# etemesi254/zune-jpeg

Hardware: AMD Instinct MI355X
Metric: megapixels/sec decoded (IDCT->RGB), 4K 4:2:0 baseline (higher is better)
Workload: dtype i32

## Files before the change

zune-jpeg_amd/csrc/zj_device.h:

```cpp
#pragma once

#include <stdint.h>

#if defined(ZJ_EMU)
#define ZJ_DEV inline
#define ZJ_HD inline
#else
#include <hip/hip_runtime.h>
#define ZJ_DEV __device__ __forceinline__
#define ZJ_HD __host__ __device__ __forceinline__
#endif

namespace zj {

typedef uint16_t u16x2 __attribute__((vector_size(4)));
typedef int16_t s16x2 __attribute__((vector_size(4)));

#if defined(ZJ_EMU)
#define ZJ_GLOBAL_PTR(T, v) (reinterpret_cast<T*>(v))
#else
#define ZJ_GLOBAL_PTR(T, v) ((T*)(__attribute__((address_space(1))) T*)(v))
#endif

struct alignas(16) U4 { uint32_t x, y, z, w; };
// ... 1 lines not shown
typedef uint32_t V4 __attribute__((vector_size(16)));
#if defined(ZJ_ABLATION)
#define ZJ_ABL(debug, bit) ((debug) & (bit))
#define ZJ_PDBG(p) ((p).debug)
#else
#define ZJ_ABL(debug, bit) 0
#define ZJ_PDBG(p) 0
#endif
#ifndef ZJ_NT
#define ZJ_NT 4
#endif
#ifndef ZJ_SEAM_WB
#define ZJ_SEAM_WB 0
#endif
#ifndef ZJ_ROUND_ROT
#define ZJ_ROUND_ROT 1
#endif

#ifndef ZJ_CBYTE
#define ZJ_CBYTE 1
#endif
#ifndef ZJ_INTERIOR
#define ZJ_INTERIOR 1
#endif

ZJ_DEV uint32_t as_u32(u16x2 v) { uint32_t r; __builtin_memcpy(&r, &v, 4); return r; }
ZJ_DEV uint32_t as_u32(s16x2 v) { uint32_t r; __builtin_memcpy(&r, &v, 4); return r; }
ZJ_DEV u16x2 as_u16x2(uint32_t v) { u16x2 r; __builtin_memcpy(&r, &v, 4); return r; }
ZJ_DEV s16x2 as_s16x2(uint32_t v) { s16x2 r; __builtin_memcpy(&r, &v, 4); return r; }

#if !defined(ZJ_EMU)
extern "C" __device__ __attribute__((const)) int zj_llvm_mul_i24(int, int) __asm("llvm.amdgcn.mul.i24");
#endif
ZJ_DEV int32_t mul24(int32_t a, int32_t b)
{
#if defined(ZJ_EMU)
    int32_t a24 = (int32_t)((uint32_t)a << 8) >> 8, b24 = (int32_t)((uint32_t)b << 8) >> 8;
    return (int32_t)((uint32_t)a24 * (uint32_t)b24);
#else
    return zj_llvm_mul_i24(a, b);
#endif
}
ZJ_DEV int32_t wadd(int32_t a, int32_t b) { return (int32_t)((uint32_t)a + (uint32_t)b); }
ZJ_DEV int32_t wsub(int32_t a, int32_t b) { return (int32_t)((uint32_t)a - (uint32_t)b); }
ZJ_DEV int32_t mad24(int32_t a, int32_t b, int32_t c) { return wadd(mul24(a, b), c); }
ZJ_DEV int32_t wshl(int32_t a, int s) { return (int32_t)((uint32_t)a << s); }
// ... 283 lines not shown
ZJ_DEV PackedHalf idct_1d_dot(const uint32_t p04, const uint32_t p26, const uint32_t p13, const uint32_t p57, const int32_t bias)
{
    PackedHalf h;
    const int32_t t0 = dot2(p04, pk16(4096, 4096), bias);
    const int32_t t1 = dot2(p04, pk16(4096, -4096), bias);
    h.x0 = dot2(p26, pk16(5352, 2217), t0);
    h.x3 = dot2(p26, pk16(-5352, -2217), t0);
    h.x1 = dot2(p26, pk16(2217, -5350), t1);
    h.x2 = dot2(p26, pk16(-2217, 5350), t1);
    h.u3 = dot2(p57, pk16(3219, 1131), dot2z(p13, pk16(5683, 4816)));
    h.u2 = dot2(p57, pk16(-5681, -3218), dot2z(p13, pk16(4816, -1129)));
    h.u1 = dot2(p57, pk16(1132, 4816), dot2z(p13, pk16(3219, -5681)));
    h.u0 = dot2(p57, pk16(4816, -5680), dot2z(p13, pk16(1131, -3218)));
    return h;
}
ZJ_DEV void idct_1d_dot_add(const PackedHalf& h, int32_t o[8])
{
    o[0] = wadd(h.x0, h.u3); o[7] = wsub(h.x0, h.u3);
    o[1] = wadd(h.x1, h.u2); o[6] = wsub(h.x1, h.u2);
    o[2] = wadd(h.x2, h.u1); o[5] = wsub(h.x2, h.u1);
    o[3] = wadd(h.x3, h.u0); o[4] = wsub(h.x3, h.u0);
}

ZJ_DEV int classify_block(const uint32_t* w, const uint32_t* g)
{
    uint32_t any = w[0] & 0xffff0000u;
#pragma unroll
    for (int i = 1; i < 32; i++) any |= w[i];
    if (any == 0) return 0;
    int32_t bad = 0;
#pragma unroll
    for (int jj = 0; jj < 4; jj++) {
        uint32_t st = 0, sb = 0;
#pragma unroll
        for (int k = 0; k < 4; k++) st = sad_u16(w[4 * k + jj], 0x80008000u, st);
#pragma unroll
        for (int k = 4; k < 8; k++) sb = sad_u16(w[4 * k + jj], 0x80008000u, sb);
        const int32_t d = mad24((int32_t)g[4 + jj], (int32_t)sb, mad24((int32_t)g[jj], (int32_t)st, -(int32_t)g[8 + jj]));
        bad |= d;
    }
    return bad < 0 ? 2 : 1;
}

ZJ_DEV void idct_block_packed(const U4 raw[8], const uint32_t* qp, uint32_t out[16])
{
    const uint32_t* w = reinterpret_cast<const uint32_t*>(raw);
    uint32_t D[32];
#pragma unroll
// ... 132 lines not shown
    static constexpr int NT_BLK = (NBLK + 63) / 64 * 64;
    static constexpr int NT_MIN = (HS == 1 && VS == 1) ? (CHROMA ? ZJ_NT_MIN_444 : ZJ_NT_MIN_GRAY) : ((HS == 2 && VS == 1 && CHROMA) ? ZJ_NT_MIN_H : ((HS == 2 && VS == 2 && CHROMA) ? ZJ_NT_MIN_HV : ((HS == 1 && VS == 2 && CHROMA) ? ZJ_NT_MIN_V : 0)));
    static constexpr int NT = NT_BLK > NT_MIN ? NT_BLK : NT_MIN;
    static constexpr int NW = NT / 64;
    static constexpr int ROUND_ROT = (ZJ_ROUND_ROT && NITEMS % NT != 0 && NITEMS % NT <= 64 && NW > 1) ? 1 : 0;

    static constexpr int LUT_N = SH + 2;
    static constexpr int LUT_BYTES = ((2 * LUT_N * 2 + 15) / 16) * 16;
    static constexpr int HRAW = (CHROMA && HALO) ? 2 * 2 * CROWS : 0;
    static constexpr int HFIL = (CHROMA && HALO) ? 2 * 2 * SH : 0;
    static constexpr bool TSCAP = OUT == OUT_RGB || OUT == OUT_YCBCR || OUT == OUT_RGBA;
    static constexpr int PPI = OUT == OUT_RGBA ? 4 : 3;
    static constexpr int INPL = 64 / PPI * PPI;
    static constexpr int XSTAGE = ((64 * PPI - INPL) * 16 + 31) / 32 * 32;
    static constexpr bool HALO_PURE = CHROMA && HALO && (NYB + 2 * CBR * TWC) % 64 == 0 && 2 * CBR * 2 * 8 == 64;
    static constexpr int HALO_T0 = NYB + 2 * CBR * TWC;
#if defined(ZJ_EMU) && !defined(ZJ_EMU_REDO_ANY)
    static constexpr bool CBYTE_OUT = OUT == OUT_RGB || OUT == OUT_RGBA || OUT == OUT_RGB_CHW;
#else
    static constexpr bool CBYTE_OUT = true;
#endif
    static constexpr bool CBYTE = ZJ_CBYTE != 0 && CHROMA && HS == 2 && HALO_PURE && NGRP == 16 && NYB % 64 == 0 && CBYTE_OUT;
    static constexpr bool INTERIOR = ZJ_INTERIOR != 0 && CBYTE && TSCAP && NITEMS % NT == 0 && ROUND_ROT == 0;
    template <int GEN> struct L {
        static constexpr int YPX = GEN == GEN_PACKED ? 1 : 2;
        static constexpr bool CB = GEN == GEN_PACKED && CBYTE;
        static constexpr int CPX = CB ? 1 : 2;
        static constexpr int CPB = CPITCH * CPX;
        static constexpr int CPLANE = CROWS * CPB;
        static constexpr int CBYTES = CHROMA ? 2 * CPLANE + (HRAW + HFIL) * 2 : 0;
        static_assert(CBYTES % 16 == 0, "tables stay 16-byte aligned");
        static constexpr int C_OFF = GEN == GEN_PACKED ? (NITEMS + 63) / 64 * 64 * 16 : YSZ * 2;
        static constexpr int HRAW_OFF = C_OFF + 2 * CPLANE;
        static constexpr int HFIL_OFF = HRAW_OFF + HRAW * 2;
        static constexpr int TAB_OFF = C_OFF + CBYTES;
        static constexpr int LUT_OFF = TAB_OFF + TAB_BYTES;
        static constexpr int FLAG_OFF = LUT_OFF + LUT_BYTES;
        static constexpr int X_OFF = FLAG_OFF + 16;
        static constexpr int X_STAGE = TSCAP ? NW * XSTAGE : 0;
        static constexpr int X_HALO = HALO_PURE ? 8 * 80 * 4 : 0;
        static constexpr int BYTES = GEN == GEN_PACKED ? X_OFF + (X_STAGE > X_HALO ? X_STAGE : X_HALO) : FLAG_OFF;
        static_assert(C_OFF % 16 == 0 && TAB_OFF % 16 == 0, "16-byte alignment of the planes");
    };
    static constexpr int LDS_WIDE = L<GEN_WIDE>::BYTES;
    static constexpr int LDS_PACKED = L<GEN_PACKED>::BYTES > LDS_WIDE ? L<GEN_PACKED>::BYTES : LDS_WIDE;
    static constexpr int PIECES_PER_ROW = PPI * NGRP;
// ... 259 lines not shown
    }
    if (GEN == GEN_PACKED && tid == 0) *lds_flag<C>(lds) = 0;
}

ZJ_DEV void rows_to_bytes(const U4 px[8], uint32_t b[16])
{
#pragma unroll
    for (int r = 0; r < 8; r++) {
        b[2 * r] = perm(px[r].y, px[r].x, 0x06040200u);
        b[2 * r + 1] = perm(px[r].w, px[r].z, 0x06040200u);
    }
}
ZJ_DEV void bytes_to_rows(const uint32_t b[16], U4 px[8])
{
#pragma unroll
    for (int r = 0; r < 8; r++) {
        px[r].x = perm(0, b[2 * r], 0x0c010c00u); px[r].y = perm(0, b[2 * r], 0x0c030c02u);
        px[r].z = perm(0, b[2 * r + 1], 0x0c010c00u); px[r].w = perm(0, b[2 * r + 1], 0x0c030c02u);
    }
}

struct HaloLane { const int16_t* src; char* dst; int pitch; int comp; int hb; int j; bool last_col; };

template <class C>
ZJ_DEV HaloLane halo_locate(const Params& p, const TileId t, const int hl , char* lds)
{
    HaloLane H;
    H.hb = hl >> 3; H.j = hl & 7;
    H.comp = 1 + H.hb / (2 * C::CBR);
    const int brow = (H.hb / 2) % C::CBR, side = H.hb & 1;
    const int cbw = p.mcu_x, cb0 = t.tile * C::TWC;
    const int nvalid = (cbw - cb0) < C::TWC ? (cbw - cb0) : C::TWC;
    const int gcol = side == 0 ? (cb0 > 0 ? cb0 - 1 : cbw - 1) : (cb0 + nvalid < cbw ? cb0 + nvalid : 0);
    const long long blk = (long long)(t.strip * C::CBR + brow) * cbw + gcol;
    const int16_t* plane = H.comp == 1 ? t.cb : t.cr;
    H.src = plane + blk * 64 + H.j;
    H.dst = reinterpret_cast<char*>(lds_halo_raw<C, GEN_PACKED>(lds, H.comp, side, brow * 8));
    H.pitch = 2;
    H.last_col = side == 0;
    return H;
}
ZJ_DEV void halo_load(const HaloLane& H, int32_t s[8])
{
#pragma unroll
    for (int k = 0; k < 8; k++) s[k] = H.src[8 * k];
}
template <class C> ZJ_DEV int32_t* lds_halo_scratch(char* lds, const int hb) { return reinterpret_cast<int32_t*>(lds + C::template L<GEN_PACKED>::X_OFF) + 80 * hb; }

template <class C>
ZJ_DEV void halo_pass1(const HaloLane& H, const int32_t s[8], char* lds)
{
    const uint16_t* q = reinterpret_cast<const uint16_t*>(lds_tab<C, GEN_PACKED>(lds) + TAB_DW * H.comp);
    int32_t* sc = lds_halo_scratch<C>(lds, H.hb);
    int32_t any = H.j == 0 ? 0 : s[0];
    int32_t d[8], o[8];
#pragma unroll
// ... 30 lines not shown
        int32_t u3 = mul24(t1, 6149 + 4816 - 3685 - 1597);
        u3 = mad24(t7, 4816 - 3685, u3);
        u3 = mad24(t5, 4816 - 1597, u3);
        u3 = mad24(t3, 4816, u3);
        v = (H.last_col ? wsub(x0, u3) : wadd(x0, u3)) >> 17;
        v = v < 0 ? 0 : (v > 255 ? 255 : v);
    }
    *reinterpret_cast<int16_t*>(H.dst + i * H.pitch) = (int16_t)v;
}

template <class C, int HS, int VS, int GEN>
ZJ_DEV int halo_value(char* lds, const int comp, const int side, const int m, const bool wrap)
{
    const int16_t* raw = lds_halo_raw<C, GEN>(lds, comp, side, 0);
    if (VS == 2) {
        const int16_t* lut = lds_lut<C, GEN>(lds);
        const int i = m + 1 + (wrap ? (side == 0 ? -1 : 1) : 0);
        const int ra = lut[i] / C::template L<GEN>::CPB, rb = lut[C::LUT_N + i] / C::template L<GEN>::CPB;
        return tri1(raw[ra], raw[rb]);
    }
    const int r = side == 0 ? (wrap && m > 0 ? m - 1 : m) : (wrap && m < C::SH - 1 ? m + 1 : m);
    return raw[r];
}
template <class C, int HS, int VS>
ZJ_DEV void halo_filter(const Params& p, const TileId t, const int hl, char* lds)
{
    const int cbw = p.mcu_x, cb0 = t.tile * C::TWC;
    const bool left_wrap = cb0 == 0, right_wrap = cb0 + C::TWC >= cbw;
    for (int q = hl; q < C::HFIL; q += 64) {
        const int comp = 1 + q / (2 * C::SH), side = (q / C::SH) & 1, m = q % C::SH;
        *lds_halo_fil<C, GEN_PACKED>(lds, comp, side, m) = (int16_t)halo_value<C, HS, VS, GEN_PACKED>(lds, comp, side, m, side == 0 ? left_wrap : right_wrap);
    }
}

template <class C, int GEN, bool NEED_Y16>
ZJ_DEV void finish_block(const BlockLoc& L, const U4 raw[8], char* lds, const int debug = 0, const int clamp_dc = 0)
{
    if (!L.valid) return;
    const uint32_t* w = reinterpret_cast<const uint32_t*>(raw);
    const uint32_t* tab = lds_tab<C, GEN>(lds) + TAB_DW * L.comp;
    if (GEN == GEN_WIDE) {
        uint32_t any = w[0] & 0xffff0000u;
#pragma unroll
        for (int i = 1; i < 32; i++) any |= w[i];
        if (any != 0 && !ZJ_ABL(debug, 1)) {
            U4 px[8];
            idct_block(raw, reinterpret_cast<const uint16_t*>(tab), px);
            store_block(L, px);
        } else {
            store_splat(L, dc_only_value(w[0], (int32_t)(tab[0] & 0xffffu), clamp_dc));
        }
        return;
    }
    using LLp = typename C::template L<GEN_PACKED>;
    constexpr bool CB = LLp::CB;
    constexpr bool CONST_PITCH = C::HALO_PURE && (CB || C::TWY * LLp::YPX == LLp::CPB);
    BlockLoc Lc = L;
    if (CONST_PITCH) { Lc.pitch = LLp::CPB; Lc.halo = 0; }
    const int ypitch = CONST_PITCH ? C::TWY * LLp::YPX : L.pitch;
    int cls = classify_block(w, tab + 32);
    if (ZJ_ABL(debug, 1)) cls = 0;
    if (cls == 0) {
        const uint32_t v = dc_only_value(w[0], (int32_t)(tab[0] & 0xffffu), clamp_dc);
        if (L.comp != 0 && !CB) { store_splat(Lc, v); return; }
        if ((L.comp != 0 || NEED_Y16) && (v & 0xffffu) > 255u) *lds_flag<C>(lds) = 1;
        const uint32_t b = (v & 0xffu) * 0x01010101u;
        const U2 row = {b, b};
        if (L.comp != 0) {
#pragma unroll
            for (int r = 0; r < 8; r++) *reinterpret_cast<U2*>(Lc.dst + r * Lc.pitch) = row;
            return;
        }
#pragma unroll
        for (int r = 0; r < 8; r++) *reinterpret_cast<U2*>(Lc.dst + r * ypitch) = row;
        return;
    }
    auto emit = [&](const uint32_t* b) {
        if (L.comp == 0) {
#pragma unroll
            for (int r = 0; r < 8; r++) { const U2 row = {b[2 * r], b[2 * r + 1]}; *reinterpret_cast<U2*>(Lc.dst + r * ypitch) = row; }
        } else if (CB) {
#pragma unroll
            for (int r = 0; r < 8; r++) { const U2 row = {b[2 * r], b[2 * r + 1]}; *reinterpret_cast<U2*>(Lc.dst + r * Lc.pitch) = row; }
// ... 174 lines not shown
        prev = (uint32_t)__builtin_amdgcn_update_dpp((int)pl, (int)a1, 0x111, 0xf, 0xf, false);
        next = (uint32_t)__builtin_amdgcn_update_dpp((int)nr, (int)a0, 0x101, 0xf, 0xf, false);
        return;
    }
#endif
    prev = next = 0;
    if (g > 0) {
        prev = *reinterpret_cast<const uint32_t*>(cp + oa + lc - 4);
        if (VS == 2) prev = tri_b(prev, *reinterpret_cast<const uint32_t*>(cp + ob + lc - 4));
    }
    if (g < C::NGRP - 1) {
        next = *reinterpret_cast<const uint32_t*>(cp + oa + lc + 8);
        if (VS == 2) next = tri_b(next, *reinterpret_cast<const uint32_t*>(cp + ob + lc + 8));
    }
}

template <class C>
ZJ_DEV bool interior_tile(const Params& p, const TileId t)
{
    const int cb0 = t.tile * C::TWC;
    return cb0 != 0 && cb0 + C::TWC < p.mcu_x && p.height - t.strip * C::SH >= C::SH && p.edge_rep == 0;
}

template <class C, bool INTERIOR = false>
ZJ_DEV void stage_item(const ItemOut& io, const int tid , char* lds, const int round, const int hw_wave = -1)
{
    if (!INTERIOR && io.kind == 0) return;
    const int lwave = tid >> 6, lane = tid & 63;
    const int item0 = 64 * lwave + round * C::NT;
    const int wave = hw_wave < 0 ? lwave : hw_wave;
    if (!INTERIOR && C::PPI == 3 && io.kind == 3) {
        const U4 z = {0, 0, 0, 0};
        *reinterpret_cast<U4*>(piece_addr<C>(lds, item0, wave, 3 * lane - 1)) = io.s0;
        *reinterpret_cast<U4*>(piece_addr<C>(lds, item0, wave, 3 * lane)) = io.s1;
        *reinterpret_cast<U4*>(piece_addr<C>(lds, item0, wave, 3 * lane + 1)) = io.s2;
        *reinterpret_cast<U4*>(piece_addr<C>(lds, item0, wave, 3 * lane + 2)) = z;
        return;
    }
    U4* const dst = reinterpret_cast<U4*>(piece_addr<C>(lds, item0, wave, C::PPI * lane));
    dst[0] = io.s0;
    dst[1] = io.s1;
    if (C::PPI == 4) { dst[2] = io.s2; dst[3] = io.s3; }
    else if (INTERIOR || io.kind == 1) dst[2] = io.s2;
}

template <class C, int HS, int VS, int OUT, int GEN, bool FAST = true, bool TS = false, bool RAG = false, bool INTERIOR = false>
ZJ_DEV void phase_color(const Params& p, const TileId t, const int tid, char* lds, const int round = 0, ItemOut* io = nullptr)
{
    using LL = typename C::template L<GEN>;
    static_assert(!INTERIOR || (TS && FAST && !RAG && GEN == GEN_PACKED && LL::CB && C::INTERIOR), "the interior form exists for the staged byte-chroma rounds");
    const int P = p.mcu_x * 8 * HS;
    const int W = p.width;
    const int cbw = p.mcu_x;
    const int cb0 = t.tile * C::TWC;
    const int nvalid = INTERIOR ? C::TWC : ((cbw - cb0) < C::TWC ? (cbw - cb0) : C::TWC);
    const bool left_wrap = !INTERIOR && cb0 == 0, right_wrap = !INTERIOR && cb0 + C::TWC >= cbw;
    const bool edge_tile = HS == 2 && (left_wrap || right_wrap);
    const int x0 = t.tile * C::TWY;
    const long long row_bytes = p.out_pitch;
    uint8_t* const frame_out = t.out;
    const int elements = P / 16 - 1;
    if (TS) io->kind = 0;

    for (int item = TS ? tid + round * C::NT : tid; item < C::NITEMS; item += TS ? C::NITEMS : C::NT) {
        const int m = item / C::NGRP, g = item % C::NGRP;
        const int px0 = x0 + 16 * g;
        const int row = t.strip * C::SH + m;
        if (!INTERIOR && (px0 >= P || row >= p.height)) continue;
        const bool irregular = RAG && px0 >= p.regular_px;
        uint8_t* const orow = frame_out + (long long)row * row_bytes;
        uint32_t yp[8];
        if (GEN == GEN_PACKED) {
            const U4 yv = *reinterpret_cast<const U4*>(lds + 16 * item);
            if (OUT == OUT_GRAY) {
                if (FAST && !irregular) store16(orow + px0, yv, true);
                else { const uint32_t ow4[4] = {yv.x, yv.y, yv.z, yv.w}; store_clip(orow, px0, ow4, 4, W, 0, 0); }
                continue;
            }
            const uint32_t yb[4] = {yv.x, yv.y, yv.z, yv.w};
#pragma unroll
            for (int k = 0; k < 4; k++) {
                if (HS == 2) { yp[k] = perm(0, yb[k], 0x0c020c00u); yp[4 + k] = perm(0, yb[k], 0x0c030c01u); }
                else { yp[2 * k] = perm(0, yb[k], 0x0c010c00u); yp[2 * k + 1] = perm(0, yb[k], 0x0c030c02u); }
            }
        } else {
            const U4* yrow = reinterpret_cast<const U4*>(lds + 32 * item);
            const U4 ya = yrow[0], yb = yrow[1];
            const uint32_t yw[8] = {ya.x, ya.y, ya.z, ya.w, yb.x, yb.y, yb.z, yb.w};
            if (OUT == OUT_GRAY) {
                U4 o;
                o.x = perm(yw[1], yw[0], 0x06040200u); o.y = perm(yw[3], yw[2], 0x06040200u);
                o.z = perm(yw[5], yw[4], 0x06040200u); o.w = perm(yw[7], yw[6], 0x06040200u);
                if (FAST && !irregular) store16(orow + px0, o);
                else { const uint32_t ow4[4] = {o.x, o.y, o.z, o.w}; store_clip(orow, px0, ow4, 4, W, 0, 0); }
                continue;
            }
            if (HS == 2) {
#pragma unroll
                for (int k = 0; k < 4; k++) {
                    yp[k] = perm(yw[2 * k + 1], yw[2 * k], 0x05040100u);
                    yp[4 + k] = perm(yw[2 * k + 1], yw[2 * k], 0x07060302u);
                }
            } else {
#pragma unroll
                for (int k = 0; k < 8; k++) yp[k] = yw[k];
            }
        }

        uint32_t cbp[8], crp[8];
        bool first = false, last = false;
        int oa, ob;
        if (VS == 2) {
            const int16_t* lut = lds_lut<C, GEN>(lds);
            oa = lut[m + 1]; ob = lut[C::LUT_N + m + 1];
        } else {
            oa = ob = m * LL::CPB;
        }
        if (edge_tile) {
            ZJ_NO_IF_CONVERT();
            first = (g == 0) && left_wrap;
            last = (8 * g + 8 == 8 * nvalid) && right_wrap;
        }
        const bool rep_first = first && p.edge_rep, rep_last = last && p.edge_rep;
        const bool no_left = first && m == 0 && !p.edge_rep, no_right = last && m == C::SH - 1 && !p.edge_rep;
#pragma unroll
        for (int ch = 0; ch < 2; ch++) {
            const char* cp = lds + LL::C_OFF + ch * LL::CPLANE;
            uint32_t* dst = ch ? crp : cbp;
            if (ZJ_ABL(ZJ_PDBG(p), 16)) {
#pragma unroll
                for (int k = 0; k < 8; k++) dst[k] = yp[k] + ch;
                continue;
            }
            if (HS == 1) {
                const U4* A = reinterpret_cast<const U4*>(cp + oa + 32 * g);
                const U4 a0 = A[0], a1 = A[1];
                uint32_t v[8] = {a0.x, a0.y, a0.z, a0.w, a1.x, a1.y, a1.z, a1.w};
                if (VS == 2) {
                    const U4* B = reinterpret_cast<const U4*>(cp + ob + 32 * g);
                    const U4 b0 = B[0], b1 = B[1];
                    const uint32_t f[8] = {b0.x, b0.y, b0.z, b0.w, b1.x, b1.y, b1.z, b1.w};
#pragma unroll
                    for (int k = 0; k < 8; k++) v[k] = tri(v[k], f[k]);
                }
#pragma unroll
                for (int k = 0; k < 8; k++) dst[k] = v[k];
            } else if (LL::CB) {
// ... 11 lines not shown
                    nb_bytes<C, VS>(a0, a1, cp, oa, ob, lc, g, prev, next, pl, nr);
#if defined(ZJ_EMU)
                    constexpr bool DPP_ENDS = false;
#else
                    constexpr bool DPP_ENDS = C::NGRP == 16;
#endif
                    if (!DPP_ENDS) {
                        if (g == 0) prev = pl;
                        if (g == nvalid - 1) next = nr;
                    } else if (!INTERIOR && nvalid != C::NGRP) {
                        ZJ_NO_IF_CONVERT();
                        if (g == nvalid - 1) next = nr;
                    }
                }
                if (!INTERIOR && p.edge_rep) {
                    ZJ_NO_IF_CONVERT();
                    if (rep_first) prev = a0 << 24;
                    if (rep_last) next = a1 >> 24;
                }
                const uint32_t l0 = alignbyte(a0, prev, 3), l1 = alignbyte(a1, a0, 3);
                const uint32_t r0 = alignbyte(a1, a0, 1), r1 = alignbyte(next, a1, 1);
                uint32_t e0 = tri_b(a0, l0), e1 = tri_b(a1, l1);
                uint32_t o0 = tri_b(a0, r0), o1 = tri_b(a1, r1);
                if (edge_tile) {
                    ZJ_NO_IF_CONVERT();
                    if (no_left) e0 = (e0 & 0xffffff00u) | (a0 & 0xffu);
                    if (no_right) {
                        e1 = (e1 & 0x00ffffffu) | ((o1 << 8) & 0xff000000u);
                        o1 = (o1 & 0x00ffffffu) | (a1 & 0xff000000u);
                    }
                }
                dst[0] = perm(0, e0, 0x0c010c00u); dst[1] = perm(0, e0, 0x0c030c02u);
                dst[2] = perm(0, e1, 0x0c010c00u); dst[3] = perm(0, e1, 0x0c030c02u);
                dst[4] = perm(0, o0, 0x0c010c00u); dst[5] = perm(0, o0, 0x0c030c02u);
                dst[6] = perm(0, o1, 0x0c010c00u); dst[7] = perm(0, o1, 0x0c030c02u);
            } else {
                const int lc = (C::COFF + 8 * g) * 2;
                const U4 a = *reinterpret_cast<const U4*>(cp + oa + lc);
                uint32_t vm[4] = {a.x, a.y, a.z, a.w};
                if (VS == 2) {
                    const U4 b = *reinterpret_cast<const U4*>(cp + ob + lc);
                    vm[0] = tri(vm[0], b.x); vm[1] = tri(vm[1], b.y);
                    vm[2] = tri(vm[2], b.z); vm[3] = tri(vm[3], b.w);
                }
                uint32_t prev, next;
                {
                    int hvl, hvr;
// ... 84 lines not shown
                uint8_t* prow = orow + (long long)pl * p.plane_stride;
                if (FAST && !irregular) { const U4 v = {q[0], q[1], q[2], q[3]}; store16(prow + px0, v); }
                else store_clip(prow, px0, q, 4, W, 0, 0);
            }
            continue;
        }
        ZJ_COLOR_SB();
#pragma unroll
        for (int k = 0; k < 4; k++) {
            if (HS == 2) pack_rgb4_eo(c[k], c[4 + k], d[3 * k], d[3 * k + 1], d[3 * k + 2]);
            else pack_rgb4_nat(c[2 * k], c[2 * k + 1], d[3 * k], d[3 * k + 1], d[3 * k + 2]);
        }
        if (!FAST || (irregular && !TS)) {
#pragma unroll
            for (int h = 0; h < 2; h++) store_unit_generic<OUT>(p, orow, P, (px0 >> 3) + h, d + 6 * h);
            continue;
        }
        const U4 s0 = {d[0], d[1], d[2], d[3]}, s1 = {d[4], d[5], d[6], d[7]}, s2 = {d[8], d[9], d[10], d[11]};
        if (ZJ_ABL(ZJ_PDBG(p), 8) && (d[0] ^ d[5] ^ d[11]) != 0x12345u) continue;
        const int G = px0 >> 4;
        const bool quirk = OUT == OUT_RGB && !p.plain && !RAG;
        if (TS) {
            io->s0 = s0; io->s1 = s1; io->s2 = s2;
            io->kind = INTERIOR ? 1 : ((quirk && G == elements) ? 3 : ((quirk && G == elements - 1) ? 2 : 1));
            continue;
        }
        if (!quirk) {
            uint8_t* o = orow + 48ll * G;
            store16(o, s0); store16(o + 16, s1); store16(o + 32, s2);
        } else {
            if (G < elements - 1) {
                uint8_t* o = orow + 48ll * G;
                store16(o, s0); store16(o + 16, s1); store16(o + 32, s2);
            } else if (G == elements - 1) {
                uint8_t* o = orow + 48ll * G;
                store16(o, s0); store16(o + 16, s1);
            } else {
                uint8_t* o = orow + 3ll * W - 64;
                store16(o, s0); store16(o + 16, s1); store16(o + 32, s2);
                if (p.zero_fill) { const U4 z = {0, 0, 0, 0}; store16(o + 48, z); }
            }
        }
    }
}

template <class C, int OUT, bool RAG = false, bool SEAM = false, bool INTERIOR = false>
ZJ_DEV void color_copyout(const Params& p, const TileId t, const int tid , char* lds, const int round, const int hw_wave = -1)
{
    using LL = typename C::template L<GEN_PACKED>;
    static_assert(!INTERIOR || (!RAG && !SEAM && C::INTERIOR), "the interior form exists for the plain staged rounds");
    constexpr int PPI = C::PPI;
    const int P = RAG ? p.regular_px : p.mcu_x * 8 * (C::TWYB / C::TWC);
    const int x0 = t.tile * C::TWY;
    const int left = P - x0 > 0 ? (P - x0) / 16 : 0;
    const int nvg = left < C::NGRP ? left : C::NGRP;
    const uint32_t row_bytes = (uint32_t)p.out_pitch;
    uint8_t* const tile_out = t.out + (long long)t.strip * C::SH * row_bytes + (long long)(PPI == 4 ? 4 : 3) * x0;
    const int w = uniform(tid >> 6), L = tid & 63;
    const int item0 = 64 * w + round * C::NT;
    if (!INTERIOR && item0 >= C::NITEMS) return;
    const bool row_end_here = !RAG && x0 + 16 * nvg == P;
    const int never = (OUT == OUT_RGB && !p.plain && !p.zero_fill && row_end_here) ? 3 * nvg - 1 : -1;
    const int rows_left = p.height - t.strip * C::SH;
    const char* const ybase = lds + 16 * item0;
    const char* const xbase = lds + LL::X_OFF + C::XSTAGE * (hw_wave < 0 ? w : hw_wave) - 16 * C::INPL;
    const char* src[PPI];
    uint32_t off[PPI];
    int mm[PPI], cc[PPI];
    constexpr bool WHOLE_ROWS = C::NT % C::NGRP == 0;
    const int item_q = WHOLE_ROWS ? 64 * w : item0;
    const int row_shift = WHOLE_ROWS ? round * (C::NT / C::NGRP) : 0;
#pragma unroll
    for (int j = 0; j < PPI; j++) {
        src[j] = (j == 0 && L < C::INPL ? ybase : xbase) + 16 * (64 * j + L);
        const int Q = PPI * item_q + 64 * j + L;
        const int m0 = (int)(((uint32_t)Q * (uint32_t)C::PPR_MAGIC) >> 20);
        cc[j] = Q - m0 * C::PIECES_PER_ROW;
        mm[j] = m0 + row_shift;
        off[j] = (uint32_t)mul24(m0, (int32_t)row_bytes) + 16u * (uint32_t)cc[j] + (uint32_t)row_shift * row_bytes;
    }
    const bool plain_round = INTERIOR || (nvg == C::NGRP && rows_left >= C::SH && never < 0 && item0 + 64 <= C::NITEMS);
    static_assert(!(SEAM && RAG), "the seam form serves aligned widths");
    uint32_t la0 = 0, lrho = 0, segb = 0;
    if (SEAM) { la0 = (uint32_t)reinterpret_cast<uintptr_t>(tile_out) & 127u; lrho = row_bytes & 127u; segb = 16u * (uint32_t)(PPI * nvg); }
    const bool seams = SEAM && (la0 | lrho) != 0;
    auto shared_line = [&](const int j) {
        const uint32_t A = (la0 + (uint32_t)mm[j] * lrho) & 127u, ls = (A + 16u * (uint32_t)cc[j]) & ~127u;
        return ls < A || ls + 128u > A + segb;
    };
    if (RAG) {
        const uint32_t a0 = (uint32_t)reinterpret_cast<uintptr_t>(tile_out) & 3u, rho = row_bytes & 3u;
        if ((a0 | rho) != 0) {
            ZJ_NO_IF_CONVERT();
#pragma unroll
            for (int j = 0; j < PPI; j++) {
                const bool ok = plain_round || (PPI * item0 + 64 * j + L < PPI * C::NITEMS && cc[j] < PPI * nvg && mm[j] < rows_left);
                const bool last = cc[j] == PPI * nvg - 1;
                const uint32_t delta = (4u - ((a0 + (uint32_t)mm[j] * rho) & 3u)) & 3u;
                const U4 v = *reinterpret_cast<const U4*>(src[j]);
                const int qn = 64 * j + L + 1;
                const char* const src2 = last ? src[j] : (qn < C::INPL ? ybase : xbase) + 16 * qn;
                const uint32_t nx = *reinterpret_cast<const uint32_t*>(src2);
// ... 225 lines not shown
```

zune-jpeg_amd/csrc/zj_kernels.hip:

```cpp
#include <hip/hip_runtime.h>
#include <atomic>
#include <stdio.h>

#include "zj_device.h"
#include "zj_launch.h"

#ifndef ZJ_WAVES_PER_SIMD
#define ZJ_WAVES_PER_SIMD 5
#endif
#ifndef ZJ_WAVES_PER_SIMD_PACKED
#define ZJ_WAVES_PER_SIMD_PACKED 6
#endif

namespace zj {

#ifndef ZJ_PRIO
#define ZJ_PRIO 1
#endif
#define ZJ_SETPRIO(bit, level) do { if (ZJ_PRIO & (bit)) __builtin_amdgcn_s_setprio(level); } while (0)

template <class C, int HS, int VS, int OUT, bool FAST, bool RAG = false>
__device__ __forceinline__ void tile_wide(const Params& p, const TileId t, const int tid, char* lds)
{
    ZJ_SETPRIO(1, 3);
    const BlockLoc L = locate<C, GEN_WIDE>(p, t, tid, lds);
    U4 raw[8];
    load_block(L, raw, ZJ_PDBG(p));
    ZJ_SETPRIO(1, 0);
    phase_setup<C, HS, VS, GEN_WIDE>(p, tid, lds);
    __syncthreads();
    finish_block<C, GEN_WIDE, false>(L, raw, lds, ZJ_PDBG(p), p.clamp_dc);
    __syncthreads();
    ZJ_SETPRIO(2, 2);
    phase_color<C, HS, VS, OUT, GEN_WIDE, FAST, false, RAG>(p, t, tid, lds);
}

template <class C, int HS, int VS, int OUT>
__device__ __forceinline__ void interior_rounds(const Params& p, const TileId t, const int tid, char* lds)
{
    static_assert(C::ROUND_ROT == 0, "full rounds: the logical thread numbering is the hardware's");
    __builtin_assume(tid >= 0 && tid < C::NT);
#pragma unroll
    for (int round = 0; round * C::NT < C::NITEMS; round++) {
        ItemOut io;
        phase_color<C, HS, VS, OUT, GEN_PACKED, true, true, false, true>(p, t, tid, lds, round, &io);
        if (round == 0 && ZJ_ABL(ZJ_PDBG(p), 128)) { ZJ_USE(io.s0.x ^ io.s0.y ^ io.s0.z ^ io.s0.w ^ io.s1.x ^ io.s1.y ^ io.s1.z ^ io.s1.w ^ io.s2.x ^ io.s2.y ^ io.s2.z ^ io.s2.w); return; }
        stage_item<C, true>(io, tid, lds, round);
        ZJ_WAVE_FENCE();
        color_copyout<C, OUT, false, false, true>(p, t, tid, lds, round);
        ZJ_WAVE_FENCE();
        if (round == 0 && ZJ_ABL(ZJ_PDBG(p), 256)) return;
    }
}

__device__ __forceinline__ void stagger_start(const Params& p, const int bid)
{
    if (p.stagger_delay <= 0 || bid >= p.stagger_wgs) return;
    const Magic g = {p.stagger_magic, p.stagger_shift};
    const int k = (int)magic_div((uint32_t)bid, g);
    const int n = k * p.stagger_delay;
    for (int i = 0; i < n; i++) __builtin_amdgcn_s_sleep(2);
}

#ifndef ZJ_ASSUME_NO_HALO
#define ZJ_ASSUME_NO_HALO 1
#endif
#ifndef ZJ_PIN_ARGS
#define ZJ_PIN_ARGS 1
#endif
__device__ __forceinline__ void pin_head(const Params& p)
{
    if (!ZJ_PIN_ARGS) return;
    asm volatile("; kernel arguments 0x00-0x87 are resident"
                 :: "s"(p.y), "s"(p.cb), "s"(p.cr), "s"(p.out), "s"(p.y_frame_stride), "s"(p.c_frame_stride), "s"(p.out_frame_stride),
                    "s"(p.width), "s"(p.height), "s"(p.mcu_x), "s"(p.n_strips), "s"(p.tiles_per_row), "s"(p.regular_px), "s"(p.zero_fill),
                    "s"(p.total_tiles), "s"(p.tpr_magic), "s"(p.tpr_shift), "s"(p.ns_magic), "s"(p.ns_shift), "s"(p.stagger_wgs),
                    "s"(p.stagger_delay), "s"(p.stagger_magic), "s"(p.stagger_shift), "s"(p.plain), "s"(p.out_pitch));
}

template <int HS, int VS, int OUT, int GEN, bool FAST, bool TS, bool RAG, bool SEAM = false>
__device__ __forceinline__ void fused_body(const Params& p, char* lds)
{
    using C = Cfg<HS, VS, OUT>;
    pin_head(p);
    const TileId t = decode_tile(p, (int)blockIdx.x);
#ifndef ZJ_ROTATE
#define ZJ_ROTATE 0
#endif
#ifndef ZJ_ROLE_SHIFT
#define ZJ_ROLE_SHIFT 0
#endif
    int tid = (int)threadIdx.x;
    if ((ZJ_ROTATE || ZJ_ROLE_SHIFT) && C::NW > 1) {
        const unsigned b = blockIdx.x;
        const int rot = ZJ_ROTATE ? (int)((b ^ (b >> 3) ^ (b >> 8)) % (unsigned)C::NW) : ZJ_ROLE_SHIFT % C::NW;
        tid += 64 * rot;
        if ((C::NT & (C::NT - 1)) == 0) tid &= C::NT - 1; else if (tid >= C::NT) tid -= C::NT;
        __builtin_assume(tid >= 0 && tid < C::NT);
    }
    stagger_start(p, (int)blockIdx.x);
    if (GEN == GEN_WIDE) { tile_wide<C, HS, VS, OUT, FAST, RAG>(p, t, tid, lds); return; }
    constexpr bool NEED_Y16 = OUT == OUT_RGB || OUT == OUT_RGBA || OUT == OUT_RGB_CHW;
    ZJ_SETPRIO(1, 3);
    const bool halo_wave = C::HALO_PURE && (__builtin_amdgcn_readfirstlane(tid) >> 6) == C::HALO_T0 / 64;
    if (halo_wave) {
        HaloLane H = halo_locate<C>(p, t, tid - C::HALO_T0, lds);
        int32_t hs8[8];
        halo_load(H, hs8);
        ZJ_SETPRIO(1, 0);
        phase_setup<C, HS, VS, GEN_PACKED>(p, tid, lds);
        if (ZJ_ABL(ZJ_PDBG(p), 32)) return;
        __syncthreads();
        halo_pass1<C>(H, hs8, lds);
        ZJ_WAVE_FENCE();
        halo_pass2<C>(H, lds, p.clamp_dc);
        ZJ_WAVE_FENCE();
        halo_filter<C, HS, VS>(p, t, tid - C::HALO_T0, lds);
    } else {
        if (ZJ_ASSUME_NO_HALO && C::HALO_PURE && C::NT == C::HALO_T0 + 64) __builtin_assume(tid < C::HALO_T0);
        const BlockLoc L = locate<C, GEN_PACKED>(p, t, tid, lds);
        U4 raw[8];
        load_block(L, raw, ZJ_PDBG(p));
        ZJ_SETPRIO(1, 0);
        phase_setup<C, HS, VS, GEN_PACKED>(p, tid, lds);
        if (ZJ_ABL(ZJ_PDBG(p), 32)) return;
        __syncthreads();
        finish_block<C, GEN_PACKED, NEED_Y16>(L, raw, lds, ZJ_PDBG(p), p.clamp_dc);
    }
    __builtin_amdgcn_s_waitcnt(0x0f70);
    if (ZJ_ABL(ZJ_PDBG(p), 64)) return;
    __syncthreads();
    const bool redo = (NEED_Y16 || C::CBYTE) && __builtin_amdgcn_readfirstlane((int)*lds_flag<C>(lds)) != 0;
    if (redo) {
        __syncthreads();
        tile_wide<C, HS, VS, OUT, FAST, RAG>(p, t, tid, lds);
    } else if (TS) {
        ZJ_SETPRIO(2, 2);
        __builtin_amdgcn_s_waitcnt(0x0f70);
        constexpr bool INTERIOR = C::INTERIOR && FAST && !RAG && !SEAM;
        if constexpr (INTERIOR) {
            if (interior_tile<C>(p, t)) { interior_rounds<C, HS, VS, OUT>(p, t, tid, lds); return; }
        }
#pragma unroll
        for (int round = 0; round * C::NT < C::NITEMS; round++) {
            ItemOut io;
            const int hw = C::ROUND_ROT ? uniform(tid >> 6) : -1, ltid = round_tid<C>(tid, round);
            phase_color<C, HS, VS, OUT, GEN_PACKED, FAST, true, RAG>(p, t, ltid, lds, round, &io);
            if (round == 0 && ZJ_ABL(ZJ_PDBG(p), 128)) { ZJ_USE(io.s0.x ^ io.s0.y ^ io.s0.z ^ io.s0.w ^ io.s1.x ^ io.s1.y ^ io.s1.z ^ io.s1.w ^ io.s2.x ^ io.s2.y ^ io.s2.z ^ io.s2.w); return; }
            stage_item<C>(io, ltid, lds, round, hw);
            ZJ_WAVE_FENCE();
            color_copyout<C, OUT, RAG, SEAM>(p, t, ltid, lds, round, hw);
            ZJ_WAVE_FENCE();
            if (round == 0 && ZJ_ABL(ZJ_PDBG(p), 256)) return;
        }
    } else {
        ZJ_SETPRIO(2, 2);
        __builtin_amdgcn_s_waitcnt(0x0f70);
        phase_color<C, HS, VS, OUT, GEN_PACKED, FAST, false, RAG>(p, t, tid, lds);
    }
}

template <int HS, int VS, int OUT, int GEN, bool FAST, bool TS>
__global__ __launch_bounds__((Cfg<HS, VS, OUT>::NT), (GEN == GEN_PACKED ? ZJ_WAVES_PER_SIMD_PACKED : ZJ_WAVES_PER_SIMD)) void zj_fused_kernel(const Params p)
{
// ... 298 lines not shown
```

Baseline: 988,100.

## Add specialized first/last row-end tile forms and interior halo path

Adds FORM_FIRST and FORM_LAST specializations of the color/stage/copyout path so tiles at the left and right image edges use compile-time edge handling instead of the general branchy path. The halo wave also gets an interior variant that drops the wrap and bounds logic. Alternative classify-sum and AND-unpack paths are added but disabled by default. The cost is more template instantiations, which means larger code and possible instruction-cache or register pressure.

```diff
diff --git a/zune-jpeg_amd/csrc/zj_device.h b/zune-jpeg_amd/csrc/zj_device.h
--- a/zune-jpeg_amd/csrc/zj_device.h
+++ b/zune-jpeg_amd/csrc/zj_device.h
@@ -47,6 +47,18 @@
 #endif
 #ifndef ZJ_INTERIOR
 #define ZJ_INTERIOR 1
+#endif
+#ifndef ZJ_ROWEND
+#define ZJ_ROWEND 1
+#endif
+#ifndef ZJ_HALO_INTERIOR
+#define ZJ_HALO_INTERIOR 1
+#endif
+#ifndef ZJ_CLASSIFY_SUMS
+#define ZJ_CLASSIFY_SUMS 0
+#endif
+#ifndef ZJ_UNPACK_AND
+#define ZJ_UNPACK_AND 0
 #endif
 
 ZJ_DEV uint32_t as_u32(u16x2 v) { uint32_t r; __builtin_memcpy(&r, &v, 4); return r; }
@@ -376,8 +388,27 @@
     o[3] = wadd(h.x3, h.u0); o[4] = wsub(h.x3, h.u0);
 }
 
+template <bool SUMS = false>
 ZJ_DEV int classify_block(const uint32_t* w, const uint32_t* g)
 {
+    if (SUMS && ZJ_CLASSIFY_SUMS) {
+        uint32_t st[4], sb[4];
+#pragma unroll
+        for (int jj = 0; jj < 4; jj++) {
+            st[jj] = sb[jj] = 0;
+#pragma unroll
+            for (int k = 0; k < 4; k++) st[jj] = sad_u16(w[4 * k + jj], 0x80008000u, st[jj]);
+#pragma unroll
+            for (int k = 4; k < 8; k++) sb[jj] = sad_u16(w[4 * k + jj], 0x80008000u, sb[jj]);
+        }
+        const uint32_t all = ((st[0] + st[1] + st[2]) + (st[3] + sb[0] + sb[1])) + (sb[2] + sb[3]);
+        const uint32_t dc = sad_u16(w[0] & 0xffffu, 0x00008000u, 8u * 262144u - 32768u);
+        if (all == dc) return 0;
+        int32_t bad = 0;
+#pragma unroll
+        for (int jj = 0; jj < 4; jj++) bad |= mad24((int32_t)g[4 + jj], (int32_t)sb[jj], mad24((int32_t)g[jj], (int32_t)st[jj], -(int32_t)g[8 + jj]));
+        return bad < 0 ? 2 : 1;
+    }
     uint32_t any = w[0] & 0xffff0000u;
 #pragma unroll
     for (int i = 1; i < 32; i++) any |= w[i];
@@ -556,6 +587,7 @@
 #endif
     static constexpr bool CBYTE = ZJ_CBYTE != 0 && CHROMA && HS == 2 && HALO_PURE && NGRP == 16 && NYB % 64 == 0 && CBYTE_OUT;
     static constexpr bool INTERIOR = ZJ_INTERIOR != 0 && CBYTE && TSCAP && NITEMS % NT == 0 && ROUND_ROT == 0;
+    static constexpr bool ROWEND = ZJ_ROWEND != 0 && INTERIOR && NGRP == 16;
     template <int GEN> struct L {
         static constexpr int YPX = GEN == GEN_PACKED ? 1 : 2;
         static constexpr bool CB = GEN == GEN_PACKED && CBYTE;
@@ -861,7 +893,7 @@
 
 struct HaloLane { const int16_t* src; char* dst; int pitch; int comp; int hb; int j; bool last_col; };
 
-template <class C>
+template <class C, bool INTERIOR = false>
 ZJ_DEV HaloLane halo_locate(const Params& p, const TileId t, const int hl , char* lds)
 {
     HaloLane H;
@@ -869,8 +901,9 @@
     H.comp = 1 + H.hb / (2 * C::CBR);
     const int brow = (H.hb / 2) % C::CBR, side = H.hb & 1;
     const int cbw = p.mcu_x, cb0 = t.tile * C::TWC;
-    const int nvalid = (cbw - cb0) < C::TWC ? (cbw - cb0) : C::TWC;
-    const int gcol = side == 0 ? (cb0 > 0 ? cb0 - 1 : cbw - 1) : (cb0 + nvalid < cbw ? cb0 + nvalid : 0);
+    const int nvalid = INTERIOR ? C::TWC : ((cbw - cb0) < C::TWC ? (cbw - cb0) : C::TWC);
+    const int gcol = INTERIOR ? (side == 0 ? cb0 - 1 : cb0 + C::TWC)
+                              : (side == 0 ? (cb0 > 0 ? cb0 - 1 : cbw - 1) : (cb0 + nvalid < cbw ? cb0 + nvalid : 0));
     const long long blk = (long long)(t.strip * C::CBR + brow) * cbw + gcol;
     const int16_t* plane = H.comp == 1 ? t.cb : t.cr;
     H.src = plane + blk * 64 + H.j;
@@ -947,18 +980,18 @@
     const int r = side == 0 ? (wrap && m > 0 ? m - 1 : m) : (wrap && m < C::SH - 1 ? m + 1 : m);
     return raw[r];
 }
-template <class C, int HS, int VS>
+template <class C, int HS, int VS, bool INTERIOR = false>
 ZJ_DEV void halo_filter(const Params& p, const TileId t, const int hl, char* lds)
 {
     const int cbw = p.mcu_x, cb0 = t.tile * C::TWC;
-    const bool left_wrap = cb0 == 0, right_wrap = cb0 + C::TWC >= cbw;
+    const bool left_wrap = !INTERIOR && cb0 == 0, right_wrap = !INTERIOR && cb0 + C::TWC >= cbw;
     for (int q = hl; q < C::HFIL; q += 64) {
         const int comp = 1 + q / (2 * C::SH), side = (q / C::SH) & 1, m = q % C::SH;
         *lds_halo_fil<C, GEN_PACKED>(lds, comp, side, m) = (int16_t)halo_value<C, HS, VS, GEN_PACKED>(lds, comp, side, m, side == 0 ? left_wrap : right_wrap);
     }
 }
 
-template <class C, int GEN, bool NEED_Y16>
+template <class C, int GEN, bool NEED_Y16, bool SUMS = false>
 ZJ_DEV void finish_block(const BlockLoc& L, const U4 raw[8], char* lds, const int debug = 0, const int clamp_dc = 0)
 {
     if (!L.valid) return;
@@ -983,7 +1016,7 @@
     BlockLoc Lc = L;
     if (CONST_PITCH) { Lc.pitch = LLp::CPB; Lc.halo = 0; }
     const int ypitch = CONST_PITCH ? C::TWY * LLp::YPX : L.pitch;
-    int cls = classify_block(w, tab + 32);
+    int cls = classify_block<SUMS>(w, tab + 32);
     if (ZJ_ABL(debug, 1)) cls = 0;
     if (cls == 0) {
         const uint32_t v = dc_only_value(w[0], (int32_t)(tab[0] & 0xffffu), clamp_dc);
@@ -1204,10 +1237,24 @@
     return cb0 != 0 && cb0 + C::TWC < p.mcu_x && p.height - t.strip * C::SH >= C::SH && p.edge_rep == 0;
 }
 
-template <class C, bool INTERIOR = false>
+enum { FORM_GENERAL = 0, FORM_INTERIOR = 1, FORM_FIRST = 2, FORM_LAST = 3 };
+
+template <class C, int OUT>
+ZJ_DEV int rowend_form(const Params& p, const TileId t)
+{
+    const int cb0 = t.tile * C::TWC;
+    if (p.height - t.strip * C::SH < C::SH || p.edge_rep != 0 || p.mcu_x <= C::TWC) return FORM_GENERAL;
+    if (cb0 == 0) return FORM_FIRST;
+    if (cb0 + C::TWC == p.mcu_x && !(OUT == OUT_RGB && p.plain)) return FORM_LAST;
+    return FORM_GENERAL;
+}
+
+template <class C, int FORM = FORM_GENERAL>
 ZJ_DEV void stage_item(const ItemOut& io, const int tid , char* lds, const int round, const int hw_wave = -1)
 {
-    if (!INTERIOR && io.kind == 0) return;
+    constexpr bool INTERIOR = FORM == FORM_INTERIOR || FORM == FORM_FIRST;
+    static_assert(FORM != FORM_LAST || C::PPI == 3, "only the RGB tail makes a last tile's staging differ from an interior one's");
+    if (FORM == FORM_GENERAL && io.kind == 0) return;
     const int lwave = tid >> 6, lane = tid & 63;
     const int item0 = 64 * lwave + round * C::NT;
     const int wave = hw_wave < 0 ? lwave : hw_wave;
@@ -1226,23 +1273,28 @@
     else if (INTERIOR || io.kind == 1) dst[2] = io.s2;
 }
 
-template <class C, int HS, int VS, int OUT, int GEN, bool FAST = true, bool TS = false, bool RAG = false, bool INTERIOR = false>
+template <class C, int HS, int VS, int OUT, int GEN, bool FAST = true, bool TS = false, bool RAG = false, int FORM = FORM_GENERAL>
 ZJ_DEV void phase_color(const Params& p, const TileId t, const int tid, char* lds, const int round = 0, ItemOut* io = nullptr)
 {
     using LL = typename C::template L<GEN>;
+    constexpr bool INTERIOR = FORM != FORM_GENERAL;
     static_assert(!INTERIOR || (TS && FAST && !RAG && GEN == GEN_PACKED && LL::CB && C::INTERIOR), "the interior form exists for the staged byte-chroma rounds");
+    static_assert(FORM == FORM_GENERAL || FORM == FORM_INTERIOR || C::ROWEND, "the row-end forms exist where Cfg::ROWEND says so");
     const int P = p.mcu_x * 8 * HS;
     const int W = p.width;
     const int cbw = p.mcu_x;
     const int cb0 = t.tile * C::TWC;
     const int nvalid = INTERIOR ? C::TWC : ((cbw - cb0) < C::TWC ? (cbw - cb0) : C::TWC);
-    const bool left_wrap = !INTERIOR && cb0 == 0, right_wrap = !INTERIOR && cb0 + C::TWC >= cbw;
+    const bool left_wrap = FORM == FORM_FIRST || (!INTERIOR && cb0 == 0), right_wrap = FORM == FORM_LAST || (!INTERIOR && cb0 + C::TWC >= cbw);
     const bool edge_tile = HS == 2 && (left_wrap || right_wrap);
     const int x0 = t.tile * C::TWY;
     const long long row_bytes = p.out_pitch;
     uint8_t* const frame_out = t.out;
     const int elements = P / 16 - 1;
     if (TS) io->kind = 0;
+    constexpr bool UNPACK_AND = ZJ_UNPACK_AND != 0 && GEN == GEN_PACKED && HS == 2 && TS && FAST && !RAG && C::INTERIOR;
+    uint32_t even_mask = 0x00ff00ffu;
+    if (UNPACK_AND) ZJ_PIN(even_mask);
 
     for (int item = TS ? tid + round * C::NT : tid; item < C::NITEMS; item += TS ? C::NITEMS : C::NT) {
         const int m = item / C::NGRP, g = item % C::NGRP;
@@ -1262,7 +1314,7 @@
             const uint32_t yb[4] = {yv.x, yv.y, yv.z, yv.w};
 #pragma unroll
             for (int k = 0; k < 4; k++) {
-                if (HS == 2) { yp[k] = perm(0, yb[k], 0x0c020c00u); yp[4 + k] = perm(0, yb[k], 0x0c030c01u); }
+                if (HS == 2) { yp[k] = UNPACK_AND ? (yb[k] & even_mask) : perm(0, yb[k], 0x0c020c00u); yp[4 + k] = perm(0, yb[k], 0x0c030c01u); }
                 else { yp[2 * k] = perm(0, yb[k], 0x0c010c00u); yp[2 * k + 1] = perm(0, yb[k], 0x0c030c02u); }
             }
         } else {
@@ -1298,13 +1350,16 @@
         } else {
             oa = ob = m * LL::CPB;
         }
-        if (edge_tile) {
+        if (FORM == FORM_FIRST) first = g == 0;
+        else if (FORM == FORM_LAST) last = g == C::NGRP - 1;
+        else if (edge_tile) {
             ZJ_NO_IF_CONVERT();
             first = (g == 0) && left_wrap;
             last = (8 * g + 8 == 8 * nvalid) && right_wrap;
         }
-        const bool rep_first = first && p.edge_rep, rep_last = last && p.edge_rep;
-        const bool no_left = first && m == 0 && !p.edge_rep, no_right = last && m == C::SH - 1 && !p.edge_rep;
+        const int edge_rep = INTERIOR ? 0 : p.edge_rep;
+        const bool rep_first = first && edge_rep, rep_last = last && edge_rep;
+        const bool no_left = first && m == 0 && !edge_rep, no_right = last && m == C::SH - 1 && !edge_rep;
 #pragma unroll
         for (int ch = 0; ch < 2; ch++) {
             const char* cp = lds + LL::C_OFF + ch * LL::CPLANE;
@@ -1362,7 +1417,14 @@
                 const uint32_t r0 = alignbyte(a1, a0, 1), r1 = alignbyte(next, a1, 1);
                 uint32_t e0 = tri_b(a0, l0), e1 = tri_b(a1, l1);
                 uint32_t o0 = tri_b(a0, r0), o1 = tri_b(a1, r1);
-                if (edge_tile) {
+                if (FORM == FORM_FIRST) {
+                    if (no_left) e0 = (e0 & 0xffffff00u) | (a0 & 0xffu);
+                } else if (FORM == FORM_LAST) {
+                    if (no_right) {
+                        e1 = (e1 & 0x00ffffffu) | ((o1 << 8) & 0xff000000u);
+                        o1 = (o1 & 0x00ffffffu) | (a1 & 0xff000000u);
+                    }
+                } else if (edge_tile) {
                     ZJ_NO_IF_CONVERT();
                     if (no_left) e0 = (e0 & 0xffffff00u) | (a0 & 0xffu);
                     if (no_right) {
@@ -1493,7 +1555,8 @@
         const bool quirk = OUT == OUT_RGB && !p.plain && !RAG;
         if (TS) {
             io->s0 = s0; io->s1 = s1; io->s2 = s2;
-            io->kind = INTERIOR ? 1 : ((quirk && G == elements) ? 3 : ((quirk && G == elements - 1) ? 2 : 1));
+            if (FORM == FORM_LAST) io->kind = OUT != OUT_RGB ? 1 : (g == C::NGRP - 1 ? 3 : (g == C::NGRP - 2 ? 2 : 1));
+            else io->kind = INTERIOR ? 1 : ((quirk && G == elements) ? 3 : ((quirk && G == elements - 1) ? 2 : 1));
             continue;
         }
         if (!quirk) {
@@ -1515,11 +1578,13 @@
     }
 }
 
-template <class C, int OUT, bool RAG = false, bool SEAM = false, bool INTERIOR = false>
+template <class C, int OUT, bool RAG = false, bool SEAM = false, int FORM = FORM_GENERAL>
 ZJ_DEV void color_copyout(const Params& p, const TileId t, const int tid , char* lds, const int round, const int hw_wave = -1)
 {
     using LL = typename C::template L<GEN_PACKED>;
-    static_assert(!INTERIOR || (!RAG && !SEAM && C::INTERIOR), "the interior form exists for the plain staged rounds");
+    constexpr bool INTERIOR = FORM == FORM_INTERIOR;
+    static_assert(FORM == FORM_GENERAL || (!RAG && !SEAM && C::INTERIOR), "the interior form exists for the plain staged rounds");
+    static_assert(FORM == FORM_GENERAL || FORM == FORM_INTERIOR || (FORM == FORM_LAST && OUT == OUT_RGB && C::ROWEND), "the one row-end form with a copy-out of its own");
     constexpr int PPI = C::PPI;
     const int P = RAG ? p.regular_px : p.mcu_x * 8 * (C::TWYB / C::TWC);
     const int x0 = t.tile * C::TWY;
@@ -1529,7 +1594,7 @@
     uint8_t* const tile_out = t.out + (long long)t.strip * C::SH * row_bytes + (long long)(PPI == 4 ? 4 : 3) * x0;
     const int w = uniform(tid >> 6), L = tid & 63;
     const int item0 = 64 * w + round * C::NT;
-    if (!INTERIOR && item0 >= C::NITEMS) return;
+    if (FORM == FORM_GENERAL && item0 >= C::NITEMS) return;
     const bool row_end_here = !RAG && x0 + 16 * nvg == P;
     const int never = (OUT == OUT_RGB && !p.plain && !p.zero_fill && row_end_here) ? 3 * nvg - 1 : -1;
     const int rows_left = p.height - t.strip * C::SH;
@@ -1549,6 +1614,15 @@
         cc[j] = Q - m0 * C::PIECES_PER_ROW;
         mm[j] = m0 + row_shift;
         off[j] = (uint32_t)mul24(m0, (int32_t)row_bytes) + 16u * (uint32_t)cc[j] + (uint32_t)row_shift * row_bytes;
+    }
+    if (FORM == FORM_LAST) {
+        const int skip = p.zero_fill ? -1 : PPI * C::NGRP - 1;
+        U4 v[PPI];
+#pragma unroll
+        for (int j = 0; j < PPI; j++) v[j] = *reinterpret_cast<const U4*>(src[j]);
+#pragma unroll
+        for (int j = 0; j < PPI; j++) if (cc[j] != skip) store16(tile_out + off[j], v[j], true);
+        return;
     }
     const bool plain_round = INTERIOR || (nvg == C::NGRP && rows_left >= C::SH && never < 0 && item0 + 64 <= C::NITEMS);
     static_assert(!(SEAM && RAG), "the seam form serves aligned widths");
diff --git a/zune-jpeg_amd/csrc/zj_kernels.hip b/zune-jpeg_amd/csrc/zj_kernels.hip
--- a/zune-jpeg_amd/csrc/zj_kernels.hip
+++ b/zune-jpeg_amd/csrc/zj_kernels.hip
@@ -35,19 +35,20 @@
     phase_color<C, HS, VS, OUT, GEN_WIDE, FAST, false, RAG>(p, t, tid, lds);
 }
 
-template <class C, int HS, int VS, int OUT>
+template <class C, int HS, int VS, int OUT, int FORM = FORM_INTERIOR>
 __device__ __forceinline__ void interior_rounds(const Params& p, const TileId t, const int tid, char* lds)
 {
     static_assert(C::ROUND_ROT == 0, "full rounds: the logical thread numbering is the hardware's");
+    constexpr int SFORM = (FORM == FORM_LAST && OUT == OUT_RGB) ? FORM_LAST : FORM_INTERIOR;
     __builtin_assume(tid >= 0 && tid < C::NT);
 #pragma unroll
     for (int round = 0; round * C::NT < C::NITEMS; round++) {
         ItemOut io;
-        phase_color<C, HS, VS, OUT, GEN_PACKED, true, true, false, true>(p, t, tid, lds, round, &io);
+        phase_color<C, HS, VS, OUT, GEN_PACKED, true, true, false, FORM>(p, t, tid, lds, round, &io);
         if (round == 0 && ZJ_ABL(ZJ_PDBG(p), 128)) { ZJ_USE(io.s0.x ^ io.s0.y ^ io.s0.z ^ io.s0.w ^ io.s1.x ^ io.s1.y ^ io.s1.z ^ io.s1.w ^ io.s2.x ^ io.s2.y ^ io.s2.z ^ io.s2.w); return; }
-        stage_item<C, true>(io, tid, lds, round);
+        stage_item<C, SFORM>(io, tid, lds, round);
         ZJ_WAVE_FENCE();
-        color_copyout<C, OUT, false, false, true>(p, t, tid, lds, round);
+        color_copyout<C, OUT, false, false, SFORM>(p, t, tid, lds, round);
         ZJ_WAVE_FENCE();
         if (round == 0 && ZJ_ABL(ZJ_PDBG(p), 256)) return;
     }
@@ -76,6 +77,24 @@
                     "s"(p.width), "s"(p.height), "s"(p.mcu_x), "s"(p.n_strips), "s"(p.tiles_per_row), "s"(p.regular_px), "s"(p.zero_fill),
                     "s"(p.total_tiles), "s"(p.tpr_magic), "s"(p.tpr_shift), "s"(p.ns_magic), "s"(p.ns_shift), "s"(p.stagger_wgs),
                     "s"(p.stagger_delay), "s"(p.stagger_magic), "s"(p.stagger_shift), "s"(p.plain), "s"(p.out_pitch));
+}
+
+template <class C, int HS, int VS, bool INTERIOR>
+__device__ __forceinline__ bool halo_wave_body(const Params& p, const TileId t, const int tid, char* lds)
+{
+    HaloLane H = halo_locate<C, INTERIOR>(p, t, tid - C::HALO_T0, lds);
+    int32_t hs8[8];
+    halo_load(H, hs8);
+    ZJ_SETPRIO(1, 0);
+    phase_setup<C, HS, VS, GEN_PACKED>(p, tid, lds);
+    if (ZJ_ABL(ZJ_PDBG(p), 32)) return true;
+    __syncthreads();
+    halo_pass1<C>(H, hs8, lds);
+    ZJ_WAVE_FENCE();
+    halo_pass2<C>(H, lds, p.clamp_dc);
+    ZJ_WAVE_FENCE();
+    halo_filter<C, HS, VS, INTERIOR>(p, t, tid - C::HALO_T0, lds);
+    return false;
 }
 
 template <int HS, int VS, int OUT, int GEN, bool FAST, bool TS, bool RAG, bool SEAM = false>
@@ -103,19 +122,16 @@
     constexpr bool NEED_Y16 = OUT == OUT_RGB || OUT == OUT_RGBA || OUT == OUT_RGB_CHW;
     ZJ_SETPRIO(1, 3);
     const bool halo_wave = C::HALO_PURE && (__builtin_amdgcn_readfirstlane(tid) >> 6) == C::HALO_T0 / 64;
+    constexpr bool FORMS = C::INTERIOR && FAST && TS && !RAG && !SEAM;
     if (halo_wave) {
-        HaloLane H = halo_locate<C>(p, t, tid - C::HALO_T0, lds);
-        int32_t hs8[8];
-        halo_load(H, hs8);
-        ZJ_SETPRIO(1, 0);
-        phase_setup<C, HS, VS, GEN_PACKED>(p, tid, lds);
-        if (ZJ_ABL(ZJ_PDBG(p), 32)) return;
-        __syncthreads();
-        halo_pass1<C>(H, hs8, lds);
-        ZJ_WAVE_FENCE();
-        halo_pass2<C>(H, lds, p.clamp_dc);
-        ZJ_WAVE_FENCE();
-        halo_filter<C, HS, VS>(p, t, tid - C::HALO_T0, lds);
+        bool cut;
+        if constexpr (FORMS && ZJ_HALO_INTERIOR != 0) {
+            if (interior_tile<C>(p, t)) cut = halo_wave_body<C, HS, VS, true>(p, t, tid, lds);
+            else cut = halo_wave_body<C, HS, VS, false>(p, t, tid, lds);
+        } else {
+            cut = halo_wave_body<C, HS, VS, false>(p, t, tid, lds);
+        }
+        if (cut) return;
     } else {
         if (ZJ_ASSUME_NO_HALO && C::HALO_PURE && C::NT == C::HALO_T0 + 64) __builtin_assume(tid < C::HALO_T0);
         const BlockLoc L = locate<C, GEN_PACKED>(p, t, tid, lds);
@@ -125,7 +141,7 @@
         phase_setup<C, HS, VS, GEN_PACKED>(p, tid, lds);
         if (ZJ_ABL(ZJ_PDBG(p), 32)) return;
         __syncthreads();
-        finish_block<C, GEN_PACKED, NEED_Y16>(L, raw, lds, ZJ_PDBG(p), p.clamp_dc);
+        finish_block<C, GEN_PACKED, NEED_Y16, FORMS>(L, raw, lds, ZJ_PDBG(p), p.clamp_dc);
     }
     __builtin_amdgcn_s_waitcnt(0x0f70);
     if (ZJ_ABL(ZJ_PDBG(p), 64)) return;
@@ -140,6 +156,11 @@
         constexpr bool INTERIOR = C::INTERIOR && FAST && !RAG && !SEAM;
         if constexpr (INTERIOR) {
             if (interior_tile<C>(p, t)) { interior_rounds<C, HS, VS, OUT>(p, t, tid, lds); return; }
+            if constexpr (C::ROWEND) {
+                const int form = rowend_form<C, OUT>(p, t);
+                if (form == FORM_FIRST) { interior_rounds<C, HS, VS, OUT, FORM_FIRST>(p, t, tid, lds); return; }
+                if (form == FORM_LAST) { interior_rounds<C, HS, VS, OUT, FORM_LAST>(p, t, tid, lds); return; }
+            }
         }
 #pragma unroll
         for (int round = 0; round * C::NT < C::NITEMS; round++) {
```

New measurement: 972,500. 0.984x the previous value.
